# lxa9867/ControlVAR

Measured on AMD Instinct MI355X. Metric: images/sec (256^2 autoregressive_infer_cfg, d24), higher is better.
Workload: dtype bf16; 1 GPU; ControlVAR d24 autoregressive_infer_cfg 256^2 (control+image), CFG=4.0, top_k=900, top_p=0.96, incl. 2 VQVAE decodes; synthetic weights/labels; batch_per_gpu=512, global_batch=512, seq_len=1360, parallelism=dp1 (sample-sharded, no collective)

## Files before the change

### controlvar_amd/_lib.py

```python
from __future__ import annotations

import ctypes as C
import os
import threading

HERE = os.path.dirname(os.path.abspath(__file__))
LIB_PATH = os.environ.get('CVAR_LIB') or os.path.join(HERE, 'libcvar_hip.so')
ABI_VERSION = 22

CVAR_F32, CVAR_BF16 = 0, 1
ACT_NONE, ACT_GELU_TANH, ACT_GELU_GRAD = 0, 1, 2

c_p = C.c_void_p
c_i = C.c_int
c_l = C.c_int64
c_f = C.c_float


class GemmDesc(C.Structure):
    _fields_ = [
        ('M', c_i), ('N', c_i), ('K', c_i), ('dtype', c_i),
        ('A', c_p), ('lda', c_l), ('W', c_p), ('ldw', c_l),
        ('batch', c_i),
        ('strideA', c_l), ('strideW', c_l), ('strideC', c_l), ('strideR', c_l),
        ('conv', c_i), ('Hin', c_i), ('Win', c_i), ('Cin', c_i), ('Hout', c_i), ('Wout', c_i), ('stride', c_i), ('up', c_i),
        ('alpha', c_f), ('bias', c_p), ('act', c_i),
        ('gate', c_p), ('ldg', c_l), ('gate_rows', c_i),
        ('residual', c_p), ('res_dtype', c_i), ('ldr', c_l),
        ('C', c_p), ('out_dtype', c_i), ('ldc', c_l),
        ('remap_l', c_i), ('remap_L', c_i), ('remap_off', c_i),
        ('pre_act', c_p), ('aux', c_p), ('gate_scale', c_p),
        ('ws', c_p), ('ws_bytes', c_l), ('tile_cfg', c_i), ('stagger', c_i), ('group_m', c_i),
        ('C_split', c_p), ('split_n', c_i), ('ld_split', c_l), ('split_alpha', c_f),
        ('ln_out', c_p), ('ln_out_dtype', c_i), ('ln_scale', c_p), ('ln_shift', c_p), ('ld_ln', c_l), ('ln_rows', c_i), ('ln_eps', c_f),
        ('gn_part', c_p),
    ]


SIGNATURES = {
    'cvar_abi_version': (c_i, []),
    'cvar_status_str': (C.c_char_p, [c_i]),
    'cvar_gemm': (c_i, [C.POINTER(GemmDesc), c_p]),
    'cvar_resample_u8': (c_i, [c_p, c_i, c_i, c_i, c_i, c_i, c_p, c_p, c_i, c_p, c_p]),
# ... 105 lines not shown
```

### controlvar_amd/csrc/attn.hip

```cpp
#include "cvar_common.h"
#include <type_traits>

constexpr int CVAR_ATTN_MAX_LVL = 32;

struct AttnParams {
    const void* qkv;
    const void* q;
    int ldkv, k_col, v_col, ldq, q_rows, q_pos0;
    void* out;
    int R, H, Lmax, q_off, l;
    float scale;
    int n_lvl;
    int lvl_end[CVAR_ATTN_MAX_LVL];
    int hole_lo[CVAR_ATTN_MAX_LVL], hole_hi[CVAR_ATTN_MAX_LVL];
    float* lse;
};

struct Vis { int kvlen, hlo, hhi; };
template <typename P>
__device__ __forceinline__ Vis vis_of(const P& p, int pos) {
    Vis v;
    if (p.n_lvl == 0) { v.kvlen = p.q_off + p.l; v.hlo = v.hhi = 0x7fffffff; return v; }
    int k = p.n_lvl - 1;
    for (int i = p.n_lvl - 1; i >= 0; --i)
// ... 83 lines not shown
            const float m_new = fmaxf(m, tmax);
            const float alpha = __expf(m - m_new);
            lsum *= alpha;
#pragma unroll
            for (int d = 0; d < D; ++d) o[d] *= alpha;
#pragma unroll
            for (int kk = 0; kk < KT; ++kk) {
                float pr = __expf(s[kk] - m_new);
                lsum += pr;
                if constexpr (sizeof(T) == 2) pr = bf16_to_f32(f32_to_bf16(pr));
#pragma unroll
                for (int d = 0; d < D; d += 4) {
                    const f32x4_t vv = *(const f32x4_t*)&Vs[kk][d];
                    o[d] = fmaf(pr, vv[0], o[d]); o[d + 1] = fmaf(pr, vv[1], o[d + 1]);
                    o[d + 2] = fmaf(pr, vv[2], o[d + 2]); o[d + 3] = fmaf(pr, vv[3], o[d + 3]);
                }
            }
            m = m_new;
        }
        __syncthreads();
    }
    if (valid) {
        const float inv = 1.0f / lsum;
        T* op = (T*)p.out + (r * p.l + qi) * (long)(p.H * D) + h * D;
#pragma unroll
        for (int d = 0; d < D; ++d) Elem<T>::st(op + d, o[d] * inv);
        if (p.lse) p.lse[(r * p.H + h) * (long)p.l + qi] = m + logf(lsum);
    }
}

template <bool HOLES, bool QPRE> __global__ __launch_bounds__(256) __attribute__((amdgpu_waves_per_eu(3, 3))) void attn_mfma_bf16_kernel(const AttnParams p);
template <bool HOLES> __global__ __launch_bounds__(256) __attribute__((amdgpu_waves_per_eu(3, 3))) void attn_mfma_bf16_v1_kernel(const AttnParams p);
template <bool HOLES> __global__ __launch_bounds__(256) __attribute__((amdgpu_waves_per_eu(2, 2))) void attn_mfma_bf16_q64_kernel(const AttnParams p);
#ifndef CVAR_ATTN_Q64
#define CVAR_ATTN_Q64 1
#endif
#ifndef CVAR_ATTN_Q64_MINL
#define CVAR_ATTN_Q64_MINL 192
#endif

template <typename P>
static int fill_levels(P& p, const int* lvl_end_host, int n_lvl, const int* hole_host) {
    if (n_lvl < 0 || n_lvl > CVAR_ATTN_MAX_LVL || (n_lvl > 0 && !lvl_end_host)) return CVAR_EINVAL;
    p.n_lvl = n_lvl;
    int prev = 0;
    for (int i = 0; i < CVAR_ATTN_MAX_LVL; ++i) {
        p.lvl_end[i] = i < n_lvl ? lvl_end_host[i] : 0;
        p.hole_lo[i] = p.hole_hi[i] = 0x7fffffff;
        if (i < n_lvl) {
            if (p.lvl_end[i] <= prev) return CVAR_EINVAL;
            if (hole_host && hole_host[2 * i + 1] > hole_host[2 * i]) {
                if (hole_host[2 * i] < 0 || hole_host[2 * i + 1] > prev) return CVAR_EINVAL;
                p.hole_lo[i] = hole_host[2 * i]; p.hole_hi[i] = hole_host[2 * i + 1];
            }
            prev = p.lvl_end[i];
        }
    }
    return CVAR_OK;
}

static int cvar_attention_impl(const void* qkv, const void* q, int dtype, int R, int H, int Lmax, int q_off, int l, float scale,
                               const int* lvl_end_host, int n_lvl, const int* hole_host, void* out, float* lse, void* stream, int impl) {
    if (!qkv || !out || R <= 0 || H <= 0 || l <= 0 || q_off < 0 || q_off + l > Lmax) return CVAR_EINVAL;
    AttnParams p;
    const int C = H * 64;
    if (q) {
        p.q = q; p.ldq = C; p.q_rows = l; p.q_pos0 = q_off; p.ldkv = 2 * C; p.k_col = 0; p.v_col = C;
    } else {
        p.q = qkv; p.ldq = 3 * C; p.q_rows = Lmax; p.q_pos0 = 0; p.ldkv = 3 * C; p.k_col = C; p.v_col = 2 * C;
    }
    p.qkv = qkv; p.out = out; p.R = R; p.H = H; p.Lmax = Lmax; p.q_off = q_off; p.l = l; p.scale = scale; p.lse = lse;
    { const int rc = fill_levels(p, lvl_end_host, n_lvl, hole_host); if (rc != CVAR_OK) return rc; }
    const bool qpre = (impl & 4) != 0;
    impl &= 3;
    if (qpre && (dtype != CVAR_BF16 || impl == 1 || !q)) return CVAR_EUNSUPPORTED;
    if (qpre)
        for (int i = 0; i < p.n_lvl; ++i)
            if (p.hole_lo[i] <= 0 && p.hole_hi[i] >= 64) return CVAR_EUNSUPPORTED;
    if (dtype == CVAR_BF16 && impl != 1) {
        bool holes = false;
        for (int i = 0; i < p.n_lvl; ++i) holes = holes || p.hole_lo[i] < p.hole_hi[i];
        if (impl == 2) {
            if (qpre) return CVAR_EUNSUPPORTED;
            if (holes) hipLaunchKernelGGL(attn_mfma_bf16_v1_kernel<true>, dim3(cdiv(l, 128), H, R), dim3(256), 0, as_stream(stream), p);
            else hipLaunchKernelGGL(attn_mfma_bf16_v1_kernel<false>, dim3(cdiv(l, 128), H, R), dim3(256), 0, as_stream(stream), p);
            CVAR_CHECK_LAUNCH();
            return CVAR_OK;
        }
        const long nblk = (long)cdiv(l, 128) * H * R;
        if (nblk > 0x7fffffffL) return CVAR_EUNSUPPORTED;
        const dim3 grid((unsigned)nblk), block(256);
        if (CVAR_ATTN_Q64 && qpre && l >= CVAR_ATTN_Q64_MINL && cdiv(l, 256) * 256 - l < 64 && (long)cdiv(l, 256) * H * R >= 512) {
            const dim3 grid64((unsigned)((long)cdiv(l, 256) * H * R));
            if (holes) hipLaunchKernelGGL((attn_mfma_bf16_q64_kernel<true>), grid64, block, 0, as_stream(stream), p);
            else hipLaunchKernelGGL((attn_mfma_bf16_q64_kernel<false>), grid64, block, 0, as_stream(stream), p);
            CVAR_CHECK_LAUNCH();
            return CVAR_OK;
        }
        if (holes) { if (qpre) hipLaunchKernelGGL((attn_mfma_bf16_kernel<true, true>), grid, block, 0, as_stream(stream), p);
                     else hipLaunchKernelGGL((attn_mfma_bf16_kernel<true, false>), grid, block, 0, as_stream(stream), p); }
        else { if (qpre) hipLaunchKernelGGL((attn_mfma_bf16_kernel<false, true>), grid, block, 0, as_stream(stream), p);
               else hipLaunchKernelGGL((attn_mfma_bf16_kernel<false, false>), grid, block, 0, as_stream(stream), p); }
        CVAR_CHECK_LAUNCH();
        return CVAR_OK;
    }
    dim3 grid(cdiv(l, 256), H, R), block(256);
    if (dtype == CVAR_BF16) hipLaunchKernelGGL(attn_rowwise_kernel<bf16_t>, grid, block, 0, as_stream(stream), p);
    else if (dtype == CVAR_F32) hipLaunchKernelGGL(attn_rowwise_kernel<float>, grid, block, 0, as_stream(stream), p);
    else return CVAR_EUNSUPPORTED;
    CVAR_CHECK_LAUNCH();
    return CVAR_OK;
}

constexpr float FA_M_FLOOR = -1.0e30f;
constexpr int FA_VT_STRIDE = 68;

template <bool HOLES>
__global__ __launch_bounds__(256) __attribute__((amdgpu_waves_per_eu(3, 3))) void attn_mfma_bf16_v1_kernel(const AttnParams p) {
    constexpr int D = 64, KT = 64;
    __shared__ __attribute__((aligned(16))) char Ks[KT * 128];
    __shared__ __attribute__((aligned(16))) bf16_t Vt[D * FA_VT_STRIDE];
    const int tid = threadIdx.x, lane = tid & 63, w = tid >> 6;
    const int lrow = lane & 31, hi = lane >> 5, sw = (lane >> 1) & 7;
    const int h = blockIdx.y;
// ... 542 lines not shown
        }
        __syncthreads();
    };
    typedef std::integral_constant<bool, true> Yes;
    typedef std::integral_constant<bool, false> No;
    load_tile(0);
    int kt0 = 0;
    const int wg_min_kv = range_full_prefix(p, p.q_off + min(qb * 256, p.l - 1), p.q_off + min(p.l, (qb + 1) * 256) - 1);
    if (KT <= wg_min_kv) tile(0, No{}, Yes{}); else tile(0, Yes{}, Yes{});
    kt0 = KT;
    for (; kt0 + KT <= wg_min_kv && kt0 < kv_end; kt0 += KT) tile(kt0, No{}, No{});
    for (; kt0 < kv_end; kt0 += KT) tile(kt0, Yes{}, No{});
#pragma unroll
    for (int g = 0; g < G; ++g) {
        const float ls = lsum[g] + __shfl_xor(lsum[g], 32, 64);
        if (qi[g] < p.l) {
            if (p.lse && hi == 0) p.lse[(r * p.H + h) * (long)p.l + qi[g]] = (m[g] + log2f(ls)) * 0.6931471805599453f;
            const float inv = 1.0f / ls;
            bf16_t* op = (bf16_t*)p.out + (r * p.l + qi[g]) * (long)(p.H * D) + h * D;
#pragma unroll
            for (int db = 0; db < 2; ++db)
#pragma unroll
                for (int gg = 0; gg < 4; ++gg) {
                    float ov[4];
#pragma unroll
                    for (int e = 0; e < 4; ++e) ov[e] = o[g][db][4 * gg + e] * inv;
                    *(bf16x4_t*)(op + 32 * db + 8 * gg + 4 * hi) = pack_bf16x4(ov);
                }
        }
    }
}



extern "C" int cvar_attention_rowwise(const void* qkv, const void* q, int dtype, int R, int H, int Lmax, int q_off, int l, float scale,
                                      const int* lvl_end_host, int n_lvl, const int* hole_host, void* out, float* lse, void* stream) {
    return cvar_attention_impl(qkv, q, dtype, R, H, Lmax, q_off, l, scale, lvl_end_host, n_lvl, hole_host, out, lse, stream, 1);
}
extern "C" int cvar_attention(const void* qkv, const void* q, int dtype, int R, int H, int Lmax, int q_off, int l, float scale,
                              const int* lvl_end_host, int n_lvl, const int* hole_host, void* out, float* lse, void* stream) {
    return cvar_attention_impl(qkv, q, dtype, R, H, Lmax, q_off, l, scale, lvl_end_host, n_lvl, hole_host, out, lse, stream, 0);
}
extern "C" int cvar_attention_prescaled(const void* kv, const void* q, int dtype, int R, int H, int Lmax, int q_off, int l,
                                        const int* lvl_end_host, int n_lvl, const int* hole_host, void* out, float* lse, void* stream) {
    return cvar_attention_impl(kv, q, dtype, R, H, Lmax, q_off, l, 1.0f, lvl_end_host, n_lvl, hole_host, out, lse, stream, 4);
}
extern "C" int cvar_attention_v1(const void* qkv, const void* q, int dtype, int R, int H, int Lmax, int q_off, int l, float scale,
                                 const int* lvl_end_host, int n_lvl, const int* hole_host, void* out, float* lse, void* stream) {
    return cvar_attention_impl(qkv, q, dtype, R, H, Lmax, q_off, l, scale, lvl_end_host, n_lvl, hole_host, out, lse, stream, 2);
}

struct AttnBwdParams {
    const void* qkv; const void* o; const void* dout; const float* lse; float* dsum; void* dqkv;
    int R, H, Lmax, q_off, l;
    float scale;
    int n_lvl;
    int lvl_end[CVAR_ATTN_MAX_LVL];
    int hole_lo[CVAR_ATTN_MAX_LVL], hole_hi[CVAR_ATTN_MAX_LVL];
};
__device__ __forceinline__ int kv_len_of_b(const AttnBwdParams& p, int pos) { return vis_of(p, pos).kvlen; }
__device__ __forceinline__ int first_query_of(const AttnBwdParams& p, int key) {
    if (p.n_lvl == 0) return 0;
    int b = 0;
    for (int k = 0; k < p.n_lvl; ++k) { if (key < p.lvl_end[k]) break; b = p.lvl_end[k]; }
    return max(0, b - p.q_off);
}

template <typename T>
__global__ void attn_bwd_prep_kernel(const AttnBwdParams p) {
    const long i = (long)blockIdx.x * blockDim.x + threadIdx.x;
    const long total = (long)p.R * p.l * p.H;
    if (i >= total) return;
    const int h = (int)(i % p.H);
    const long rq = i / p.H;
    const T* op = (const T*)p.o + rq * (long)(p.H * 64) + h * 64;
    const T* dp = (const T*)p.dout + rq * (long)(p.H * 64) + h * 64;
    float a[4] = {0.f, 0.f, 0.f, 0.f};
#pragma unroll
// ... 504 lines not shown
```

### controlvar_amd/models.py

```python
from __future__ import annotations

import math
from typing import Any, Dict, List, Optional, Sequence, Tuple, Union

import numpy as np
import torch
import torch.nn as nn

from . import ops
from ._lib import CvarError
from ._lib import ACT_GELU_TANH
from .pyramid import packed_tables
from .spec import DEFAULT_PATCH_NUMS, VaeConfig, check_latent_size, VarConfig, attention_levels, vae_state_shapes, var_state_shapes
from .synth import synth_vae_state, synth_var_state


class _Tree(nn.Module):
    """plain container so that dotted state_dict keys map onto nested attributes"""


def _register_tree(root: nn.Module, shapes, values: Dict[str, torch.Tensor], requires_grad: bool):
    for key, (shape, kind) in shapes.items():
        parts = key.split('.')
        m = root
# ... 692 lines not shown
    coef = np.zeros((nstage, B, 4), dtype=np.float32)
    for si in range(nstage):
        ratio = si / (nstage - 1)
        for b in range(B):
            if four_way:
                t1, t2, t3 = [c * ratio for c in cfg_r[b].tolist()]
                coef[si, b] = [1 + t1, t2 - t1, t3 - t2, -t3]
            else:
                t = float(cfg_r[b]) * ratio
                coef[si, b, :2] = [1 + t, -t]
    tab.coef.copy_(torch.from_numpy(coef))
    return tab


def _refuse_request_keywords(g_seed, request: dict):
    if request:
        raise TypeError(f'run() got {", ".join(sorted(request))}: this graph was captured with per_request=False, which bakes cfg, top_k and top_p into its '
                        'launches - capture it with per_request=True to pass them per call and per row')
    if g_seed is not None and _host_array(g_seed).ndim != 0:
        raise ValueError('g_seed: one integer - this graph was captured with per_request=False; capture it with per_request=True for one seed per row')


class ControlVAR(nn.Module):
    _control = True

    def __init__(self, vae_local: VQVAE, num_classes=1000, norm_eps=1e-6, aln=1, aln_gamma_init=1e-3, shared_aln=False,
                 cond_drop_rate=0.1, depth=16, embed_dim=1024, num_heads=16, mlp_ratio=4., drop_rate=0., attn_drop_rate=0.,
                 drop_path_rate=0., layer_scale=-1., tau=4, cos_attn=False, patch_nums=DEFAULT_PATCH_NUMS,
                 flash_if_available=True, fused_if_available=True, mask_factor=2, bidirectional=False, separate_decoding=False,
                 separator=False, type_pos=False, indep=True, multi_cond=False,
                 compute_dtype=None, init_seed: int = 0, deterministic_plan: bool = False, sampler: str = 'counter'):
        super().__init__()
        self.deterministic_plan = bool(deterministic_plan)
        self.sampler = sampler
        self._rng: Optional[torch.Generator] = None
        self._rng_assigned = False
        if separator and not (self._control and mask_factor == 2):
            raise NotImplementedError('separator needs the joint (control, image) sequence')
        if separator and len(patch_nums) != 10:
            raise NotImplementedError('separator: upstream hard-codes 18 special tokens (control_var.py:543)')
        if separate_decoding and not (self._control and mask_factor == 2):
            raise NotImplementedError('separate_decoding needs the joint (control, image) sequence')
        if bidirectional and not (self._control and mask_factor == 2):
            raise NotImplementedError('bidirectional needs the joint (control, image) sequence')
        sa_block = aln < 0
        if type_pos and not (self._control and mask_factor == 2):
            raise NotImplementedError('type_pos needs the joint (control, image) sequence: upstream builds type_1L with 2*sum(pn^2) entries')
        if self._control and mask_factor == 2 and not multi_cond:
            raise NotImplementedError('mask_factor=2 requires multi_cond=True (every shipped config)')
        if embed_dim // num_heads != 64:
            raise NotImplementedError('head_dim must be 64')
        self.cfg = VarConfig(depth=depth, mask_factor=mask_factor, multi_cond=bool(multi_cond) and self._control and mask_factor == 2,
                             control=self._control, patch_nums=tuple(patch_nums), vocab=vae_local.vocab_size, cvae=vae_local.Cvae,
                             num_classes=num_classes, embed_dim=embed_dim, num_heads=num_heads, norm_eps=norm_eps, tau=float(tau),
                             cos_attn=bool(cos_attn), mlp_ratio=mlp_ratio, cond_drop_rate=cond_drop_rate, drop_path_rate=float(drop_path_rate),
                             shared_aln=bool(shared_aln) and not sa_block, type_pos=bool(type_pos), sa_block=sa_block,
                             layer_scale=float(layer_scale) if sa_block else -1.0, bidirectional=bool(bidirectional),
                             separate_decoding=bool(separate_decoding), indep=bool(indep) and self._control and mask_factor == 2,
                             separator=bool(separator))
        self.separate_decoding, self.indep, self.separator, self.type_pos = self.cfg.separate_decoding, bool(indep), self.cfg.separator, self.cfg.type_pos
        cfg = self.cfg
        self.bidirectional = cfg.bidirectional
        self.Cvae, self.V = cfg.cvae, cfg.vocab
        self.depth, self.C, self.D, self.num_heads = depth, cfg.C, cfg.C, cfg.H
        if cfg.C > 2048:
            raise ValueError(f'embed_dim {cfg.C} > 2048: the adaLN kernels of controlvar_amd hold one row per wave (depth <= 32)')
# ... 209 lines not shown
        key = (R, Lmax, self.compute_dtype)
        if self._arena is None:
            self._arena = {}
        ent = self._arena.get(sid)
        if ent is None or ent[0] != key:
            ent = self._arena[sid] = (key, torch.empty(self.cfg.depth, R, Lmax, 2 * self.cfg.C, device=self.device, dtype=self.compute_dtype))
        return ent[1]

    def _blocks_and_head(self, x, ada, R: int, l: int, q_off: int, Lmax: int, arena, lvl_end=None, holes=None):
        P, cfg = self._pack(), self.cfg
        C, H, T = cfg.C, cfg.H, self.compute_dtype
        M = R * l
        hid = P['w_fc1'].shape[1]
        n_ada = P['n_ada']
        dev = x.device
        u = torch.empty(M, C, device=dev, dtype=T)
        o = torch.empty(M, C, device=dev, dtype=T)
        hbuf = torch.empty(M, hid, device=dev, dtype=T)
        qs = torch.empty(M, C, device=dev, dtype=T)
        arena_stride = R * Lmax * 2 * C
        LOG2E = 1.4426950408889634
        pre = T == torch.bfloat16
        q_alpha = (float(cfg.attn_scale) * LOG2E) if (pre and not cfg.uses_cos_attn) else 1.0
        sm = not self.deterministic_plan
        fuse_ln = M < FUSE_LN_BELOW
        ah = cfg.depth * 6 * C
        ops.ln_modulate(x, ada, 2 * C, 4 * C, n_ada, l, u, M, C, cfg.norm_eps)
        for i in range(cfg.depth):
            a0 = i * 6 * C
            ops.gemm(u, P['w_qkv'], arena, M=M, N=3 * C, K=C, w_off=i * 3 * C * C, bias=P['b_qkv'][i], c_off=i * arena_stride,
                     ldc=2 * C, remap=(l, Lmax, q_off), split=(qs, C, C), split_alpha=q_alpha, small_m=sm, split_k=sm)
            if cfg.uses_cos_attn:
                ops.cos_qk_norm(arena, R, H, Lmax, q_off, l, P['scale_mul'], qkv_off=i * arena_stride, sm_off=i * H, q=qs, q_mul=LOG2E if pre else 1.0)
            ops.attention(arena, o, R, H, Lmax, q_off, l, float(cfg.attn_scale), lvl_end, qkv_off=i * arena_stride, holes=holes, q=qs, prescaled=pre)
            ln2 = (u, ada, a0 + 3 * C, a0 + 5 * C, n_ada, l, cfg.norm_eps)
            ops.gemm(o, P['w_proj'], x, M=M, N=C, K=C, w_off=i * C * C, bias=P['b_proj'][i], gate=ada, gate_off=a0, ldg=n_ada, gate_rows=l,
                     residual=x, ln=ln2 if fuse_ln else None, small_m=sm, split_k=sm)
            if not fuse_ln:
                ops.ln_modulate(x, *ln2[1:6], u, M, C, cfg.norm_eps)
            ops.gemm(u, P['w_fc1'], hbuf, M=M, N=hid, K=C, w_off=i * hid * C, bias=P['b_fc1'][i], act=ACT_GELU_TANH, small_m=sm, split_k=sm)
            a1 = a0 + 6 * C
            ln1 = (u, ada, a1 + 2 * C, a1 + 4 * C, n_ada, l, cfg.norm_eps) if i + 1 < cfg.depth else (u, ada, ah, ah + C, n_ada, l, cfg.norm_eps)
            ops.gemm(hbuf, P['w_fc2'], x, M=M, N=C, K=hid, w_off=i * C * hid, bias=P['b_fc2'][i], gate=ada, gate_off=a0 + C, ldg=n_ada,
                     gate_rows=l, residual=x, ln=ln1 if fuse_ln else None, small_m=sm, split_k=sm)
            if not fuse_ln:
                ops.ln_modulate(x, *ln1[1:6], u, M, C, cfg.norm_eps)
        logits = torch.empty(M, cfg.head_ld, device=dev, dtype=torch.float32)
        ops.gemm(u, P['w_head'], logits, M=M, N=cfg.head_ld, K=C, bias=P['b_head'], small_m=sm, split_k=sm)
        return logits

    def _ada(self, cond: torch.Tensor, R: int):
        P = self._pack()
        cs = torch.empty(R, self.cfg.C, device=cond.device, dtype=self.compute_dtype)
        ops.silu_cast(cond, cs)
        ada = torch.empty(R, P['n_ada'], device=cond.device, dtype=torch.float32)
        sm = not self.deterministic_plan
        ops.gemm(cs, P['w_ada'], ada, M=R, N=P['n_ada'], K=self.cfg.C, bias=P['b_ada'], small_m=sm, split_k=sm)
        return ada

    def _as_labels(self, B, label_B, seed):
        dev = self.device
        if label_B is None:
            g = torch.Generator(device='cpu').manual_seed(seed)
            label_B = torch.randint(0, self.num_classes, (B,), generator=g)
        elif isinstance(label_B, int):
            label_B = torch.full((B,), self.num_classes if label_B < 0 else label_B)
        _check_index_range(label_B, 0, self.num_classes, 'label_B')
# ... 578 lines not shown
```

### controlvar_amd/ops.py

```python
from __future__ import annotations

import ctypes as C
from typing import Optional, Sequence

import torch

from . import _lib
from ._lib import ACT_GELU_TANH, ACT_NONE, CVAR_BF16, CVAR_F32, GemmDesc, check

_DT = {torch.float32: CVAR_F32, torch.bfloat16: CVAR_BF16}

GEMM_PROFILE = None


def dt(t_or_dtype) -> int:
    d = t_or_dtype.dtype if isinstance(t_or_dtype, torch.Tensor) else t_or_dtype
    try:
        return _DT[d]
    except KeyError:
        raise TypeError(f'unsupported dtype {d}') from None


def _stream() -> int:
    return torch.cuda.current_stream().cuda_stream
# ... 115 lines not shown
        ws = ensure_splitk_workspace(A.device)
    cs = (_ptr(colsum) + 4 * colsum_off) if colsum is not None else None
    check(_lib.load().cvar_gemm_tn(_ptr(A), lda or Nn, _ptr(B), ldb or Kk, _ptr(out) + 4 * c_off, ldc or Kk, T, Nn, Kk, ws.data_ptr(), ws.numel(), cs, _stream()),
          'cvar_gemm_tn')
    return out


def ln_modulate(x: torch.Tensor, ada: torch.Tensor, scale_off: int, shift_off: int, ld_ada: int, rows_per: int,
                out: torch.Tensor, M: int, Cdim: int, eps: float):
    base = _ptr(ada)
    check(_lib.load().cvar_ln_modulate(_ptr(x), base + 4 * scale_off, base + 4 * shift_off, ld_ada, rows_per,
                                       _ptr(out), dt(out), M, Cdim, eps, _stream()), 'cvar_ln_modulate')
    return out


def silu_cast(x: torch.Tensor, out: torch.Tensor):
    check(_lib.load().cvar_silu_cast(_ptr(x), _ptr(out), dt(out), x.numel(), _stream()), 'cvar_silu_cast')
    return out


def _level_arrays(lvl_end, holes):
    n = len(lvl_end) if lvl_end else 0
    arr = (C.c_int * max(n, 1))(*(lvl_end or [0]))
    harr = None
    if holes:
        if len(holes) != n:
            raise ValueError('one (lo, hi) hole per level')
        harr = (C.c_int * (2 * n))(*[int(v) for h in holes for v in h])
    return n, arr, harr


def attention(qkv: torch.Tensor, out: torch.Tensor, R: int, H: int, Lmax: int, q_off: int, l: int, scale: float,
              lvl_end: Optional[Sequence[int]] = None, qkv_off: int = 0, rowwise: bool = False, lse: Optional[torch.Tensor] = None,
              holes: Optional[Sequence[Sequence[int]]] = None, q: Optional[torch.Tensor] = None, prescaled: bool = False, v1: bool = False):
    n, arr, harr = _level_arrays(lvl_end, holes)
    if q is not None and (q.dtype != qkv.dtype or q.numel() < R * l * H * 64):
        raise ValueError('q must hold R*l rows of H*64 elements in the arena dtype')
    if prescaled:
        if rowwise or q is None:
            raise ValueError('prescaled queries: K/V-arena form of the MFMA kernel only')
        check(_lib.load().cvar_attention_prescaled(_ptr(qkv) + qkv_off * qkv.element_size(), _ptr(q), dt(qkv), R, H, Lmax, q_off, l,
                                                   arr, n, harr, _ptr(out), _ptr(lse), _stream()), 'cvar_attention_prescaled')
        return out
    fn = _lib.load().cvar_attention_rowwise if rowwise else (_lib.load().cvar_attention_v1 if v1 else _lib.load().cvar_attention)
    check(fn(_ptr(qkv) + qkv_off * qkv.element_size(), _ptr(q), dt(qkv), R, H, Lmax, q_off, l, scale,
                                     arr, n, harr, _ptr(out), _ptr(lse), _stream()), 'cvar_attention')
    return out


def attention_bwd(qkv, o, dout, lse, dqkv, ws, R, H, Lmax, l, scale, lvl_end=None, qkv_off: int = 0, rowwise: bool = False, holes=None):
    n, arr, harr = _level_arrays(lvl_end, holes)
    fn = _lib.load().cvar_attention_bwd_rowwise if rowwise else _lib.load().cvar_attention_bwd
    check(fn(_ptr(qkv) + qkv_off * qkv.element_size(), dt(qkv), _ptr(o), _ptr(dout), _ptr(lse), R, H, Lmax, 0, l, scale,
                                         arr, n, harr, _ptr(dqkv), _ptr(ws), _stream()), 'cvar_attention_bwd')
    return dqkv


def cos_qk_norm(qkv: torch.Tensor, R: int, H: int, Lmax: int, q_off: int, l: int, scale_mul: torch.Tensor,
                qkv_off: int = 0, sm_off: int = 0, norms: Optional[torch.Tensor] = None, q: Optional[torch.Tensor] = None, q_mul: float = 1.0):
    check(_lib.load().cvar_cos_qk_norm(_ptr(qkv) + qkv_off * qkv.element_size(), _ptr(q), dt(qkv), R, H, Lmax, q_off, l,
                                       _ptr(scale_mul) + 4 * sm_off, _ptr(norms), float(q_mul), _stream()), 'cvar_cos_qk_norm')


def cos_qk_norm_bwd(qkv, dqkv, R, H, Lmax, l, scale_mul, norms, dsm_tok, sm_off: int = 0):
    check(_lib.load().cvar_cos_qk_norm_bwd(_ptr(qkv), _ptr(dqkv), dt(qkv), R, H, Lmax, l, _ptr(scale_mul) + 4 * sm_off, _ptr(norms), _ptr(dsm_tok),
                                           _stream()), 'cvar_cos_qk_norm_bwd')


def cfg_sample(logits: torch.Tensor, B: int, nrep: int, l: int, V: int, coef: Sequence[float], top_k: int, top_p: float,
               seed: int, stage: int, n_draw: int, idx_out: torch.Tensor, combined: Optional[torch.Tensor] = None,
               margin: Optional[torch.Tensor] = None, kept: Optional[torch.Tensor] = None, seed_dev: Optional[torch.Tensor] = None,
               ldv: int = 0, codebook: Optional[torch.Tensor] = None, smooth_mul: float = 1.0, smooth_tau: float = 1.0,
               gumbel: Optional[torch.Tensor] = None, soft_out: Optional[torch.Tensor] = None, expo: Optional[torch.Tensor] = None):
    if expo is not None and (expo.dtype != torch.float32 or not expo.is_contiguous() or expo.numel() != n_draw * B * l * V
                             or expo.device != logits.device):
        raise ValueError(f'cfg_sample: expo must be a contiguous float32 ({n_draw * B}, {l}, {V}) tensor on {logits.device}')
# ... 278 lines not shown
```

### include/cvar.h

```cpp
#ifndef CVAR_H
#define CVAR_H

#include <stdint.h>

#ifdef __cplusplus
extern "C" {
#endif

typedef enum { CVAR_OK = 0, CVAR_EINVAL = -1, CVAR_EUNSUPPORTED = -2, CVAR_ELAUNCH = -3 } cvar_status;
typedef enum { CVAR_F32 = 0, CVAR_BF16 = 1 } cvar_dtype;
typedef enum { CVAR_ACT_NONE = 0, CVAR_ACT_GELU_TANH = 1, CVAR_ACT_GELU_GRAD = 2 } cvar_act;

int cvar_abi_version(void);
const char* cvar_status_str(int status);

typedef struct {
    int M, N, K;
    int dtype;
    const void* A; int64_t lda;
    const void* W; int64_t ldw;
    int batch;
    int64_t strideA, strideW, strideC, strideR;
    int conv;
    int Hin, Win, Cin, Hout, Wout, stride, up;
// ... 3 lines not shown
    const float* gate; int64_t ldg; int gate_rows;
    const void* residual; int res_dtype; int64_t ldr;
    void* C; int out_dtype; int64_t ldc;
    int remap_l, remap_L, remap_off;
    void* pre_act;
    const void* aux;
    const float* gate_scale;
    void* ws; int64_t ws_bytes;
    int tile_cfg;
    int stagger;
    int group_m;
    void* C_split; int split_n; int64_t ld_split;
    float split_alpha;
    void* ln_out; int ln_out_dtype;
    const float* ln_scale; const float* ln_shift; int64_t ld_ln; int ln_rows; float ln_eps;
    float* gn_part;
} cvar_gemm_desc;
int cvar_gemm(const cvar_gemm_desc* d, void* stream);
int cvar_conv3x3_gn_partials(int dtype, int stride, int Cin, int Cout, int Hin, int Win, int Hout, int Wout, int* tiles_per_image, int* pixels_per_tile);

int cvar_gemm_tn(const void* A, int64_t lda, const void* B, int64_t ldb, float* C, int64_t ldc, int T, int Nn, int Kk,
                 float* ws, int64_t ws_bytes, float* colsum_a, void* stream);

int cvar_ln_modulate(const float* x, const float* scale, const float* shift, int64_t ld_ada, int rows_per,
                     void* out, int out_dtype, int M, int C, float eps, void* stream);

int cvar_silu_cast(const float* x, void* out, int out_dtype, int64_t n, void* stream);

int cvar_attention(const void* qkv, const void* q, int dtype, int R, int H, int Lmax, int q_off, int l, float scale,
                   const int* lvl_end_host, int n_lvl, const int* hole_host, void* out,
                   float* lse , void* stream);
int cvar_attention_rowwise(const void* qkv, const void* q, int dtype, int R, int H, int Lmax, int q_off, int l, float scale,
                           const int* lvl_end_host, int n_lvl, const int* hole_host, void* out, float* lse, void* stream);
int cvar_attention_prescaled(const void* kv, const void* q, int dtype, int R, int H, int Lmax, int q_off, int l,
                             const int* lvl_end_host, int n_lvl, const int* hole_host, void* out, float* lse, void* stream);
int cvar_attention_v1(const void* qkv, const void* q, int dtype, int R, int H, int Lmax, int q_off, int l, float scale,
                      const int* lvl_end_host, int n_lvl, const int* hole_host, void* out, float* lse, void* stream);
int cvar_attention_bwd(const void* qkv, int dtype, const void* o, const void* dout, const float* lse, int R, int H, int Lmax,
                       int q_off, int l, float scale, const int* lvl_end_host, int n_lvl, const int* hole_host, void* dqkv, float* ws, void* stream);
int cvar_attention_bwd_rowwise(const void* qkv, int dtype, const void* o, const void* dout, const float* lse, int R, int H, int Lmax,
                               int q_off, int l, float scale, const int* lvl_end_host, int n_lvl, const int* hole_host, void* dqkv, float* ws,
                               void* stream);

int cvar_cos_qk_norm(void* qkv, void* q, int dtype, int R, int H, int Lmax, int q_off, int l, const float* scale_mul,
                     float* norms ,
                     float q_mul , void* stream);
int cvar_cos_qk_norm_bwd(const void* qkv, void* dqkv, int dtype, int R, int H, int Lmax, int l, const float* scale_mul,
                         const float* norms, float* dsm_tok, void* stream);

int cvar_cfg_sample(const float* logits, int B, int nrep, int l, int V, const float* coef_host,
                    int top_k, float top_p, uint64_t seed, const uint64_t* seed_dev , int stage, int n_draw,
                    int32_t* idx_out, float* combined, float* margin, int32_t* kept, int ldv,
                    const float* codebook , int Cvae, float smooth_mul, float smooth_tau, const float* gumbel, float* soft_out,
                    const float* expo , void* stream);

int cvar_ms_next_input(const int32_t* idx, const float* codebook, const float* phi_w, const float* phi_b,
                       const float* up_mat, const float* down_mat, float* f_hat, float* tok_out,
                       int nb, int nmaps, int pn, int pn_next, int S, int Cvae, void* stream);

int cvar_ms_encode(const float* f, const float* codebook, int V, const float* phi_w, const float* phi_b,
                   const int* phi_map_host, const int* patch_nums_host, int nscale, const float* up_mats,
                   const float* down_mats, int32_t* idx_out, float* f_hat_out, float* margin_out,
                   int B, int S, int Cvae, void* stream);

int cvar_word_embed(const float* tok, const float* W, const float* bias, const float* lvl_pos, float* x,
                    int nb, int nrep, int l, int Cvae, int C, int x_rows, int x_off, void* stream);
// ... 76 lines not shown
```

Before: 204.5 images/s.

## Add persistent work-item attention kernel packing heads for short levels

```diff
diff --git a/controlvar_amd/_lib.py b/controlvar_amd/_lib.py
--- a/controlvar_amd/_lib.py
+++ b/controlvar_amd/_lib.py
@@ -9,6 +9,12 @@
 ABI_VERSION = 22
 
 CVAR_F32, CVAR_BF16 = 0, 1
+
+
+def attn_opt(impl: int = 0, max_workgroups: int = 0) -> int:
+    return ((impl & 3) << 8) | ((max_workgroups & 0xfffff) << 12)
+
+
 ACT_NONE, ACT_GELU_TANH, ACT_GELU_GRAD = 0, 1, 2
 
 c_p = C.c_void_p
diff --git a/controlvar_amd/csrc/attn.hip b/controlvar_amd/csrc/attn.hip
--- a/controlvar_amd/csrc/attn.hip
+++ b/controlvar_amd/csrc/attn.hip
@@ -139,6 +139,8 @@
 template <bool HOLES, bool QPRE> __global__ __launch_bounds__(256) __attribute__((amdgpu_waves_per_eu(3, 3))) void attn_mfma_bf16_kernel(const AttnParams p);
 template <bool HOLES> __global__ __launch_bounds__(256) __attribute__((amdgpu_waves_per_eu(3, 3))) void attn_mfma_bf16_v1_kernel(const AttnParams p);
 template <bool HOLES> __global__ __launch_bounds__(256) __attribute__((amdgpu_waves_per_eu(2, 2))) void attn_mfma_bf16_q64_kernel(const AttnParams p);
+template <bool HOLES, int G> __global__ __launch_bounds__(256) __attribute__((amdgpu_waves_per_eu(G == 1 ? 3 : 2, G == 1 ? 3 : 2))) void attn_items_kernel(const AttnParams p, const int n_items);
+constexpr int CVAR_ATTN_ITEMS_CUS = 256;
 #ifndef CVAR_ATTN_Q64
 #define CVAR_ATTN_Q64 1
 #endif
@@ -166,8 +168,13 @@
     return CVAR_OK;
 }
 
+static bool attn_items_wins(int l, int n_items) {
+    return l <= 64 && n_items >= 512;
+}
+
 static int cvar_attention_impl(const void* qkv, const void* q, int dtype, int R, int H, int Lmax, int q_off, int l, float scale,
-                               const int* lvl_end_host, int n_lvl, const int* hole_host, void* out, float* lse, void* stream, int impl) {
+                               const int* lvl_end_host, int n_lvl, const int* hole_host, void* out, float* lse, void* stream, int impl,
+                               int items = 0, int max_workgroups = 0) {
     if (!qkv || !out || R <= 0 || H <= 0 || l <= 0 || q_off < 0 || q_off + l > Lmax) return CVAR_EINVAL;
     AttnParams p;
     const int C = H * 64;
@@ -197,6 +204,24 @@
         const long nblk = (long)cdiv(l, 128) * H * R;
         if (nblk > 0x7fffffffL) return CVAR_EUNSUPPORTED;
         const dim3 grid((unsigned)nblk), block(256);
+        if (items == 2 && !qpre) return CVAR_EUNSUPPORTED;
+        if (items == 2 && lse) return CVAR_EUNSUPPORTED;
+        if (qpre && items != 1 && !lse) {
+            const int G = l <= 32 ? 4 : l <= 64 ? 2 : 1;
+            const int n_items = G == 1 ? (int)nblk : cdiv(H * R, G);
+            if (items == 2 || attn_items_wins(l, n_items)) {
+                const int wgs = min(n_items, max_workgroups > 0 ? max_workgroups : CVAR_ATTN_ITEMS_CUS * (G == 1 ? 3 : 2));
+                const dim3 gridi((unsigned)wgs);
+                if (G == 4) { if (holes) hipLaunchKernelGGL((attn_items_kernel<true, 4>), gridi, block, 0, as_stream(stream), p, n_items);
+                              else hipLaunchKernelGGL((attn_items_kernel<false, 4>), gridi, block, 0, as_stream(stream), p, n_items); }
+                else if (G == 2) { if (holes) hipLaunchKernelGGL((attn_items_kernel<true, 2>), gridi, block, 0, as_stream(stream), p, n_items);
+                                   else hipLaunchKernelGGL((attn_items_kernel<false, 2>), gridi, block, 0, as_stream(stream), p, n_items); }
+                else { if (holes) hipLaunchKernelGGL((attn_items_kernel<true, 1>), gridi, block, 0, as_stream(stream), p, n_items);
+                       else hipLaunchKernelGGL((attn_items_kernel<false, 1>), gridi, block, 0, as_stream(stream), p, n_items); }
+                CVAR_CHECK_LAUNCH();
+                return CVAR_OK;
+            }
+        }
         if (CVAR_ATTN_Q64 && qpre && l >= CVAR_ATTN_Q64_MINL && cdiv(l, 256) * 256 - l < 64 && (long)cdiv(l, 256) * H * R >= 512) {
             const dim3 grid64((unsigned)((long)cdiv(l, 256) * H * R));
             if (holes) hipLaunchKernelGGL((attn_mfma_bf16_q64_kernel<true>), grid64, block, 0, as_stream(stream), p);
@@ -805,6 +830,218 @@
 }
 
 
+template <bool HOLES, int G>
+__global__ __launch_bounds__(256) __attribute__((amdgpu_waves_per_eu(G == 1 ? 3 : 2, G == 1 ? 3 : 2))) void attn_items_kernel(const AttnParams p, const int n_items) {
+    constexpr int D = 64, KT = 64;
+    constexpr int WPS = 4 / G, NT = 64 * WPS, QB = 32 * WPS;
+    constexpr int NI = 512 / NT, KSTEP = NT / 8;
+    constexpr int TILE_B = KT * 128;
+    __shared__ __attribute__((aligned(1024))) char KVs[G * 2 * TILE_B];
+    const int tid = threadIdx.x, lane = tid & 63;
+    const int w = __builtin_amdgcn_readfirstlane(tid >> 6);
+    const int sg = w / WPS, ws = w % WPS, ts = tid & (NT - 1);
+    char* const Ks = KVs + sg * 2 * TILE_B;
+    char* const Vs = Ks + TILE_B;
+    const int lrow = lane & 31, hi = lane >> 5, sw = (lane >> 1) & 7;
+    const int nqb = (p.l + QB - 1) / QB, pairs = p.R * p.H;
+    const int row_bytes = p.H * (4 * D);
+    const long arena_row = (long)p.Lmax * row_bytes;
+
+    auto item_of = [&](int id, int& qb, int& pair) {
+        if (G == 1) {
+            if ((pairs & 7) == 0) { const int xcd = id & 7, local = id >> 3; qb = local % nqb; pair = (local / nqb) * 8 + xcd; }
+            else { qb = id % nqb; pair = id / nqb; }
+        } else { qb = 0; pair = min(id * G + sg, pairs - 1); }
+    };
+    auto kv_end_of = [&](int qb) { return kv_len_of(p, p.q_off + min(p.l, (qb + 1) * QB) - 1); };
+    bf16x8_t qf[4];
+    auto load_q = [&](int id) {
+        int qb, pair;
+        item_of(id, qb, pair);
+        const int h = pair % p.H;
+        const long r = pair / p.H;
+        const int qrow = min(qb * QB + ws * 32 + lrow, p.l - 1);
+        const bf16_t* qp = (const bf16_t*)p.q + (r * p.l + qrow) * (long)(p.H * D) + h * D;
+#pragma unroll
+        for (int ks = 0; ks < 4; ++ks) qf[ks] = *(const bf16x8_t*)(qp + (2 * ks + hi) * 8);
+    };
+    const int k_key = ts >> 3, k_chunk = ts & 7;
+    bf16x8_t kreg[NI], vreg[NI];
+    const int ld_off = k_key * row_bytes + k_chunk * 16;
+    typedef int v4i_t __attribute__((ext_vector_type(4)));
+    auto k_of = [&](int qb, int pair) {
+        const char* kbase = (const char*)p.qkv + (pair / p.H) * arena_row + (pair % p.H) * (2 * D);
+        return __builtin_amdgcn_make_buffer_rsrc((void*)kbase, 0, (kv_end_of(qb) - 1) * row_bytes + 128, 0x00020000);
+    };
+    auto v_of = [&](int qb, int pair) {
+        const char* vbase = (const char*)p.qkv + (pair / p.H) * arena_row + (pair % p.H) * (2 * D) + (row_bytes >> 1);
+        return __builtin_amdgcn_make_buffer_rsrc((void*)vbase, 0, (kv_end_of(qb) - 1) * row_bytes + 128, 0x00020000);
+    };
+    auto load_tile = [&](const __amdgpu_buffer_rsrc_t k_rsrc, const __amdgpu_buffer_rsrc_t v_rsrc, int kt0) {
+#pragma unroll
+        for (int i = 0; i < NI; ++i) {
+            const int so = (kt0 + KSTEP * i) * row_bytes;
+            kreg[i] = __builtin_bit_cast(bf16x8_t, (v4i_t)__builtin_amdgcn_raw_buffer_load_b128(k_rsrc, ld_off, so, 0));
+            vreg[i] = __builtin_bit_cast(bf16x8_t, (v4i_t)__builtin_amdgcn_raw_buffer_load_b128(v_rsrc, ld_off, so, 0));
+        }
+    };
+    auto store_tile = [&]() {
+#pragma unroll
+        for (int i = 0; i < NI; ++i) {
+            const int key = k_key + KSTEP * i;
+            *(bf16x8_t*)(Ks + key * 128 + ((k_chunk ^ ((key >> 1) & 7)) << 4)) = kreg[i];
+            *(bf16x8_t*)(Vs + key * 128 + ((((k_chunk >> 1) ^ (key & 3)) << 5) | ((k_chunk & 1) << 4))) = vreg[i];
+        }
+    };
+    const int v_jrow = (lane & 15) >> 2, v_g = (lane >> 4) & 1;
+    const char* v_lane[2];
+#pragma unroll
+    for (int db = 0; db < 2; ++db) v_lane[db] = Vs + (4 * hi + v_jrow) * 128 + (((2 * db + v_g) ^ v_jrow) << 5) + (lane & 3) * 8;
+    const short one_bf = hi == 0 ? (short)0x3f80 : (short)0;
+    const bf16x8_t k_ones = {one_bf, 0, 0, 0, 0, 0, 0, 0};
+    typedef std::integral_constant<bool, true> Yes;
+    typedef std::integral_constant<bool, false> No;
+
+    int id = blockIdx.x;
+    if (id >= n_items) return;
+    load_q(id);
+    { int qb, pair; item_of(id, qb, pair); load_tile(k_of(qb, pair), v_of(qb, pair), 0); }
+    for (;;) {
+        const int next_id = id + (int)gridDim.x;
+        const bool has_next = next_id < n_items;
+        int qb, pair;
+        item_of(id, qb, pair);
+        const bool valid = G == 1 || id * G + sg < pairs;
+        const int h = pair % p.H;
+        const long r = pair / p.H;
+        const int q0 = qb * QB + ws * 32;
+        const bool active = q0 < p.l;
+        const int qi = q0 + lrow;
+        const Vis vis = vis_of(p, p.q_off + min(qi, p.l - 1));
+        const int kv_end = kv_end_of(qb);
+        const __amdgpu_buffer_rsrc_t k_rsrc = k_of(qb, pair), v_rsrc = v_of(qb, pair);
+        const int min_kv = range_full_prefix(p, p.q_off + min(qb * QB, p.l - 1), p.q_off + min(p.l, (qb + 1) * QB) - 1);
+
+        f32x16_t o[2];
+#pragma unroll
+        for (int db = 0; db < 2; ++db)
+#pragma unroll
+            for (int i = 0; i < 16; ++i) o[db][i] = 0.f;
+        float m = 0.f, lsum = 0.f;
+        bf16x8_t q_m = {0, 0, 0, 0, 0, 0, 0, 0};
+
+        auto tile = [&](int kt0, auto MASK, auto FIRST) {
+            store_tile();
+            __syncthreads();
+            const bool last = kt0 + KT >= kv_end;
+            if (!last) load_tile(k_rsrc, v_rsrc, kt0 + KT);
+            else if (has_next) { int nqb_, npair; item_of(next_id, nqb_, npair); load_tile(k_of(nqb_, npair), v_of(nqb_, npair), 0); }
+            f32x16_t s[2];
+            if (active) {
+#pragma unroll
+                for (int kb = 0; kb < 2; ++kb) {
+#pragma unroll
+                    for (int i = 0; i < 16; ++i) s[kb][i] = 0.f;
+                    if constexpr (!decltype(FIRST)::value) s[kb] = __builtin_amdgcn_mfma_f32_32x32x16_bf16(k_ones, q_m, s[kb], 0, 0, 0);
+#pragma unroll
+                    for (int ks = 0; ks < 4; ++ks) {
+                        const bf16x8_t kf = *(const bf16x8_t*)(Ks + (32 * kb + lrow) * 128 + (((2 * ks + hi) ^ sw) << 4));
+                        s[kb] = __builtin_amdgcn_mfma_f32_32x32x16_bf16(kf, qf[ks], s[kb], 0, 0, 0);
+                    }
+                }
+            }
+            if (last && has_next) load_q(next_id);
+            if (active) {
+                if constexpr (decltype(MASK)::value) {
+#pragma unroll
+                    for (int kb = 0; kb < 2; ++kb)
+#pragma unroll
+                        for (int i = 0; i < 16; ++i) {
+                            const int key = kt0 + 32 * kb + (i & 3) + 8 * (i >> 2) + 4 * hi;
+                            if (!vis_key_t<HOLES>(vis, key)) s[kb][i] = -INFINITY;
+                        }
+                }
+                auto row_max = [&]() {
+                    float tmax = -INFINITY;
+#pragma unroll
+                    for (int kb = 0; kb < 2; ++kb)
+#pragma unroll
+                        for (int i = 0; i < 16; ++i) tmax = fmaxf(tmax, s[kb][i]);
+                    return fmaxf(tmax, __shfl_xor(tmax, 32, 64));
+                };
+                auto shift = [&](bool always) {
+                    const float tmax = row_max();
+                    const bool need = always || tmax > 2.0f + fabsf(m) * 0.015625f;
+                    const float m_new = need ? bf16_to_f32(f32_to_bf16(m + tmax)) : m;
+                    const float delta = m_new - m;
+                    if (!always) {
+                        const float alpha = __builtin_amdgcn_exp2f(-delta);
+                        lsum *= alpha;
+#pragma unroll
+                        for (int db = 0; db < 2; ++db)
+#pragma unroll
+                            for (int i = 0; i < 16; ++i) o[db][i] *= alpha;
+                    }
+#pragma unroll
+                    for (int kb = 0; kb < 2; ++kb)
+#pragma unroll
+                        for (int i = 0; i < 16; ++i) s[kb][i] -= delta;
+                    m = m_new;
+                    q_m[0] = hi == 0 ? (short)f32_to_bf16(-m_new) : (short)0;
+                };
+                if (decltype(FIRST)::value) shift(true);
+                else if (__any(row_max() > 2.0f + fabsf(m) * 0.015625f)) shift(false);
+                bf16x8_t pf[2][2];
+#pragma unroll
+                for (int kb = 0; kb < 2; ++kb)
+#pragma unroll
+                    for (int t = 0; t < 2; ++t) {
+                        float pr[8];
+#pragma unroll
+                        for (int j = 0; j < 8; ++j) {
+                            pr[j] = __builtin_amdgcn_exp2f(s[kb][8 * t + j]);
+                            lsum += pr[j];
+                        }
+                        pf[kb][t] = pack_bf16x8(pr);
+                    }
+#pragma unroll
+                for (int db = 0; db < 2; ++db)
+#pragma unroll
+                    for (int kb = 0; kb < 2; ++kb)
+#pragma unroll
+                        for (int t = 0; t < 2; ++t) {
+                            const char* vp = v_lane[db] + (32 * kb + 16 * t) * 128;
+                            const s16x4_t v0 = lds_tr16_b64(vp);
+                            const s16x4_t v1 = lds_tr16_b64(vp + 8 * 128);
+                            const bf16x8_t vf = {v0[0], v0[1], v0[2], v0[3], v1[0], v1[1], v1[2], v1[3]};
+                            o[db] = __builtin_amdgcn_mfma_f32_32x32x16_bf16(vf, pf[kb][t], o[db], 0, 0, 0);
+                        }
+            }
+            __syncthreads();
+        };
+        if (KT <= min_kv) tile(0, No{}, Yes{}); else tile(0, Yes{}, Yes{});
+        int kt0 = KT;
+        for (; kt0 + KT <= min_kv && kt0 < kv_end; kt0 += KT) tile(kt0, No{}, No{});
+        for (; kt0 < kv_end; kt0 += KT) tile(kt0, Yes{}, No{});
+        lsum += __shfl_xor(lsum, 32, 64);
+        if (valid && qi < p.l) {
+            const float inv = 1.0f / lsum;
+            bf16_t* op = (bf16_t*)p.out + (r * p.l + qi) * (long)(p.H * D) + h * D;
+#pragma unroll
+            for (int db = 0; db < 2; ++db)
+#pragma unroll
+                for (int g = 0; g < 4; ++g) {
+                    float ov[4];
+#pragma unroll
+                    for (int e = 0; e < 4; ++e) ov[e] = o[db][4 * g + e] * inv;
+                    *(bf16x4_t*)(op + 32 * db + 8 * g + 4 * hi) = pack_bf16x4(ov);
+                }
+        }
+        if (!has_next) break;
+        id = next_id;
+    }
+}
+
 
 extern "C" int cvar_attention_rowwise(const void* qkv, const void* q, int dtype, int R, int H, int Lmax, int q_off, int l, float scale,
                                       const int* lvl_end_host, int n_lvl, const int* hole_host, void* out, float* lse, void* stream) {
@@ -816,7 +1053,9 @@
 }
 extern "C" int cvar_attention_prescaled(const void* kv, const void* q, int dtype, int R, int H, int Lmax, int q_off, int l,
                                         const int* lvl_end_host, int n_lvl, const int* hole_host, void* out, float* lse, void* stream) {
-    return cvar_attention_impl(kv, q, dtype, R, H, Lmax, q_off, l, 1.0f, lvl_end_host, n_lvl, hole_host, out, lse, stream, 4);
+    const int items = (dtype >> 8) & 3, max_workgroups = (dtype >> 12) & 0xfffff;
+    if (items == 3) return CVAR_EINVAL;
+    return cvar_attention_impl(kv, q, dtype & 0xff, R, H, Lmax, q_off, l, 1.0f, lvl_end_host, n_lvl, hole_host, out, lse, stream, 4, items, max_workgroups);
 }
 extern "C" int cvar_attention_v1(const void* qkv, const void* q, int dtype, int R, int H, int Lmax, int q_off, int l, float scale,
                                  const int* lvl_end_host, int n_lvl, const int* hole_host, void* out, float* lse, void* stream) {
diff --git a/controlvar_amd/models.py b/controlvar_amd/models.py
--- a/controlvar_amd/models.py
+++ b/controlvar_amd/models.py
@@ -748,6 +748,7 @@
                  compute_dtype=None, init_seed: int = 0, deterministic_plan: bool = False, sampler: str = 'counter'):
         super().__init__()
         self.deterministic_plan = bool(deterministic_plan)
+        self.attn_impl = 0
         self.sampler = sampler
         self._rng: Optional[torch.Generator] = None
         self._rng_assigned = False
@@ -1023,7 +1024,7 @@
                      ldc=2 * C, remap=(l, Lmax, q_off), split=(qs, C, C), split_alpha=q_alpha, small_m=sm, split_k=sm)
             if cfg.uses_cos_attn:
                 ops.cos_qk_norm(arena, R, H, Lmax, q_off, l, P['scale_mul'], qkv_off=i * arena_stride, sm_off=i * H, q=qs, q_mul=LOG2E if pre else 1.0)
-            ops.attention(arena, o, R, H, Lmax, q_off, l, float(cfg.attn_scale), lvl_end, qkv_off=i * arena_stride, holes=holes, q=qs, prescaled=pre)
+            ops.attention(arena, o, R, H, Lmax, q_off, l, float(cfg.attn_scale), lvl_end, qkv_off=i * arena_stride, holes=holes, q=qs, prescaled=pre, impl=self.attn_impl if pre else 0)
             ln2 = (u, ada, a0 + 3 * C, a0 + 5 * C, n_ada, l, cfg.norm_eps)
             ops.gemm(o, P['w_proj'], x, M=M, N=C, K=C, w_off=i * C * C, bias=P['b_proj'][i], gate=ada, gate_off=a0, ldg=n_ada, gate_rows=l,
                      residual=x, ln=ln2 if fuse_ln else None, small_m=sm, split_k=sm)
diff --git a/controlvar_amd/ops.py b/controlvar_amd/ops.py
--- a/controlvar_amd/ops.py
+++ b/controlvar_amd/ops.py
@@ -171,16 +171,21 @@
 
 def attention(qkv: torch.Tensor, out: torch.Tensor, R: int, H: int, Lmax: int, q_off: int, l: int, scale: float,
               lvl_end: Optional[Sequence[int]] = None, qkv_off: int = 0, rowwise: bool = False, lse: Optional[torch.Tensor] = None,
-              holes: Optional[Sequence[Sequence[int]]] = None, q: Optional[torch.Tensor] = None, prescaled: bool = False, v1: bool = False):
+              holes: Optional[Sequence[Sequence[int]]] = None, q: Optional[torch.Tensor] = None, prescaled: bool = False, v1: bool = False,
+              impl: int = 0, max_workgroups: int = 0):
     n, arr, harr = _level_arrays(lvl_end, holes)
     if q is not None and (q.dtype != qkv.dtype or q.numel() < R * l * H * 64):
         raise ValueError('q must hold R*l rows of H*64 elements in the arena dtype')
     if prescaled:
         if rowwise or q is None:
             raise ValueError('prescaled queries: K/V-arena form of the MFMA kernel only')
-        check(_lib.load().cvar_attention_prescaled(_ptr(qkv) + qkv_off * qkv.element_size(), _ptr(q), dt(qkv), R, H, Lmax, q_off, l,
+        if not (0 <= impl <= 2 and 0 <= max_workgroups < (1 << 20)):
+            raise ValueError('impl in 0..2, max_workgroups in [0, 2^20)')
+        check(_lib.load().cvar_attention_prescaled(_ptr(qkv) + qkv_off * qkv.element_size(), _ptr(q), dt(qkv) | _lib.attn_opt(impl, max_workgroups), R, H, Lmax, q_off, l,
                                                    arr, n, harr, _ptr(out), _ptr(lse), _stream()), 'cvar_attention_prescaled')
         return out
+    if impl or max_workgroups:
+        raise ValueError('impl / max_workgroups: prescaled queries only')
     fn = _lib.load().cvar_attention_rowwise if rowwise else (_lib.load().cvar_attention_v1 if v1 else _lib.load().cvar_attention)
     check(fn(_ptr(qkv) + qkv_off * qkv.element_size(), _ptr(q), dt(qkv), R, H, Lmax, q_off, l, scale,
                                      arr, n, harr, _ptr(out), _ptr(lse), _stream()), 'cvar_attention')
diff --git a/include/cvar.h b/include/cvar.h
--- a/include/cvar.h
+++ b/include/cvar.h
@@ -59,6 +59,7 @@
                    float* lse , void* stream);
 int cvar_attention_rowwise(const void* qkv, const void* q, int dtype, int R, int H, int Lmax, int q_off, int l, float scale,
                            const int* lvl_end_host, int n_lvl, const int* hole_host, void* out, float* lse, void* stream);
+#define CVAR_ATTN_OPT(impl, max_workgroups) ((((impl) & 3) << 8) | (((max_workgroups) & 0xfffff) << 12))
 int cvar_attention_prescaled(const void* kv, const void* q, int dtype, int R, int H, int Lmax, int q_off, int l,
                              const int* lvl_end_host, int n_lvl, const int* hole_host, void* out, float* lse, void* stream);
 int cvar_attention_v1(const void* qkv, const void* q, int dtype, int R, int H, int Lmax, int q_off, int l, float scale,
```

New measurement: 204.4 images/s. No clear change (-0.0%).
